# MatteoMer/zolt

Measured on AMD Instinct MI355X. Metric: BN254 G1 MSM/sec, higher is better.
Workload: dtype u32; 1 GPU; msm_g1_2^20; points=1048576, points_per_gpu=1048576, streams=3, window_bits=17, windows=15, table_levels=15, table_bytes=1006632960, mode=precomputed table of multiples

## Files before the change

### zolt_amd/csrc/msm.hip

```cpp
#include <string.h>

#include <mutex>
#include <vector>

#include "common.hip.h"
#include "g1.hip.h"
#include "g1_29.hip.h"
#include "g1_29x4.hip.h"
#include "msm_plan.h"

#ifndef ZG_TAIL_PRIO
#define ZG_TAIL_PRIO 3
#endif
#define ZG_HIPRIO() __builtin_amdgcn_s_setprio(ZG_TAIL_PRIO)

struct zg_bases_s {
    size_t n = 0;
    int device = -1;
    zg::MsmPlan plan;
    char *d_table = nullptr;
    uint8_t *d_inf = nullptr;
    uint64_t *d_scal = nullptr;
    struct Lane {
        uint32_t *d_dig = nullptr, *d_sorted = nullptr, *d_hist = nullptr, *d_starts = nullptr;
        uint32_t *d_blockhist = nullptr, *d_tmp = nullptr, *d_cstarts = nullptr, *d_fine = nullptr;
        zg::SortWords sort_cap;
        char *d_partial = nullptr;
        char *d_slice_buckets = nullptr;
        size_t slice_buckets = 0;
        uint32_t *d_slice_meta = nullptr;
        char *d_bits = nullptr;
        char *d_rg = nullptr;
        uint32_t *d_nzrank = nullptr;
        uint32_t *d_nzlist = nullptr;
        uint32_t *d_nzend = nullptr;
        uint32_t *d_scan_tmp = nullptr;
        char *d_part = nullptr;
        char *d_part2 = nullptr;
        uint32_t *d_heavy = nullptr;
        void *d_state = nullptr;
        hipEvent_t done = nullptr;
        hipStream_t last_st = nullptr;
        bool used = false;
    };
    std::vector<Lane> lanes;
    size_t next_lane = 0;
    Lane batch_lane;
    zg::MsmPlan batch_plan;
    size_t batch_n = 0;
    struct {
        size_t n = 0, k = 0, kc = 0;
        bool wide_ok = false;
    } fuse;
    static constexpr int NAUX = 3;
    hipStream_t aux[NAUX] = {nullptr, nullptr, nullptr};
    hipEvent_t ev_fork = nullptr, ev_join[NAUX] = {nullptr, nullptr, nullptr};
    zg_bases_s *small = nullptr;
    uint64_t *d_out = nullptr;
    uint64_t *h_out = nullptr;
    uint64_t *d_slice_parts = nullptr;
    char *d_rows_buckets = nullptr, *d_rows_bits = nullptr, *d_rows_rg = nullptr;
    size_t rows_cap = 0;
    hipEvent_t rows_done = nullptr;
    std::mutex mu;
};

namespace zg {


constexpr int PRE_GROUP = 7;
constexpr size_t PRE_CHUNK = (size_t)1 << 21;
struct PreJob {
    const uint64_t *xy;
    const uint8_t *inf;
    size_t n;
    int levels, dbl_per_level;
    char *table, *scratch;
    size_t first, count;
    unsigned blocks;
};
__global__ void __launch_bounds__(256) msm_precompute_kernel(PreJob side, PreJob main_job) {
    const bool is_side = blockIdx.x < side.blocks;
    const PreJob &jb = is_side ? side : main_job;
    const uint64_t *xy = jb.xy;
    const uint8_t *inf = jb.inf;
    const size_t n = jb.n, first = jb.first, count = jb.count;
    const int levels = jb.levels, dbl_per_level = jb.dbl_per_level;
    char *table = jb.table, *scratch = jb.scratch;
    const size_t li = (size_t)(blockIdx.x - (is_side ? 0u : side.blocks)) * blockDim.x + threadIdx.x, i = first + li;
    if (li >= count) return;
    Affine p = affine_load(xy + 8 * i);
    Jac29 a;
// ... 102 lines not shown
        __syncthreads();
    }
    if (k < NK) {
        loc[k] = sh[tid] - h;
        locz[k] = shz[tid] - z;
    }
    if (tid == 1023) {
        tile_tot[2 * blockIdx.x] = sh[1023];
        tile_tot[2 * blockIdx.x + 1] = shz[1023];
    }
}

__global__ void __launch_bounds__(1024) msm_scan_b_kernel(const uint32_t *__restrict__ hist, uint32_t NK, const uint32_t *__restrict__ loc,
                                                          const uint32_t *__restrict__ locz, const uint32_t *__restrict__ tile_tot,
                                                          uint32_t *__restrict__ starts, uint32_t *__restrict__ nzrank,
                                                          uint32_t *__restrict__ nzlist, uint32_t *__restrict__ nzend, uint32_t *__restrict__ state,
                                                          uint32_t nstate) {
    ZG_HIPRIO();
    __shared__ uint32_t pre[2];
    if (state && blockIdx.x == 0)
        for (uint32_t w = threadIdx.x; w < nstate; w += 1024) state[w] = 0;
    uint32_t tid = threadIdx.x, k = blockIdx.x * 1024 + tid;
    if (tid < 64) {
        uint32_t a = 0, az = 0;
        for (uint32_t t = tid; t < blockIdx.x; t += 64) {
            a += tile_tot[2 * t];
            az += tile_tot[2 * t + 1];
        }
        for (int d = 32; d > 0; d >>= 1) {
            a += __shfl_down(a, d, 64);
            az += __shfl_down(az, d, 64);
        }
        if (tid == 0) {
            pre[0] = a;
            pre[1] = az;
        }
    }
    __syncthreads();
    if (k < NK) {
        uint32_t s = pre[0] + loc[k], r = pre[1] + locz[k];
        starts[k] = s;
        nzrank[k] = r;
        uint32_t h = hist[k];
        if (h) {
            nzlist[r] = k;
            nzend[r] = s + h;
        }
        if (k == NK - 1) {
            starts[NK] = s + h;
            nzrank[NK] = r + (h ? 1u : 0u);
        }
    }
}

__global__ void __launch_bounds__(256) msm_scatter_kernel(const uint32_t *dig, uint32_t n, uint32_t n_pts, int G, size_t table_n,
                                                          uint32_t off, const uint32_t *starts, uint32_t *fill, uint32_t *sorted) {
    uint32_t i = blockIdx.x * 256 + threadIdx.x;
    uint32_t w = blockIdx.y;
    if (i >= n) return;
    uint32_t e = dig[(size_t)w * n + i];
    if (e == 0xFFFFFFFFu) return;
    uint32_t key = e & 0x7FFFFFFFu;
    uint32_t pos = starts[key] + atomicAdd(&fill[key], 1u);
    uint32_t ref = (uint32_t)((size_t)(w / G) * table_n + off + i % n_pts);
    sorted[pos] = (e & 0x80000000u) | ref;
}

struct RowOffs {
    uint32_t k;
    uint32_t off[33];
};
ZG_DEV void row_split(const RowOffs &r, uint32_t n_pts, uint32_t i, uint32_t &batch, uint32_t &pt) {
    if (r.k == 0) {
        batch = i / n_pts;
        pt = i - batch * n_pts;
        return;
    }
    uint32_t b = 0;
    while (b + 1 < r.k && i >= r.off[b + 1]) b++;
    batch = b;
    pt = i - r.off[b];
}

template <int C>
__global__ void __launch_bounds__(1024) msm_digits_lds_kernel(const uint64_t *scalars, const uint8_t *inf, uint32_t n, uint32_t n_pts,
                                                              int G, uint32_t per_block, uint32_t NK, int shift, uint32_t *dig,
                                                              uint32_t *blockhist, RowOffs rows) {
    ZG_HIPRIO();
    extern __shared__ uint32_t lds_hist[];
    constexpr int W = (255 + C - 1) / C;
    constexpr uint32_t NB = 1u << (C - 1);
    for (uint32_t k = threadIdx.x; k < NK; k += blockDim.x) lds_hist[k] = 0;
    __syncthreads();
    uint32_t i0 = blockIdx.x * per_block, i1 = i0 + per_block < n ? i0 + per_block : n;
    for (uint32_t i = i0 + threadIdx.x; i < i1; i += blockDim.x) {
        uint32_t batch, pt;
        row_split(rows, n_pts, i, batch, pt);
        Fr s = fr_from_mont29(fe_load<FrParams>(scalars + 4 * (rows.k ? (size_t)batch * n_pts + pt : (size_t)i)));
        bool skip = inf && inf[pt];
        uint32_t carry = 0;
#pragma unroll
        for (int w = 0; w < W; w++) {
            const int bit = w * C, limb = bit / 32, sh = bit % 32;
            uint32_t v = s.l[limb] >> sh;
            if (sh + C > 32 && limb + 1 < 8) v |= s.l[limb + 1] << (32 - sh);
            v = (v & ((1u << C) - 1u)) + carry;
            uint32_t neg = v > NB ? 1u : 0u;
            uint32_t d = neg ? (1u << C) - v : v;
            carry = neg;
            uint32_t e = 0xFFFFFFFFu;
            if (d != 0 && !skip) {
                uint32_t key = (batch * (uint32_t)G + (uint32_t)(w % G)) * NB + (d - 1);
                e = key | (neg << 31);
                atomicAdd(&lds_hist[key >> shift], 1u);
            }
            dig[(size_t)w * n + i] = e;
        }
    }
    __syncthreads();
    uint32_t *row = blockhist + (size_t)blockIdx.x * NK;
    for (uint32_t k = threadIdx.x; k < NK; k += blockDim.x) row[k] = lds_hist[k];
}

__global__ void __launch_bounds__(256) msm_colscan_kernel(uint32_t *blockhist, uint32_t nblk, uint32_t NK, uint32_t *total) {
    ZG_HIPRIO();
    uint32_t key = blockIdx.x * 256 + threadIdx.x;
    if (key >= NK) return;
    uint32_t run = 0;
    for (uint32_t b0 = 0; b0 < nblk; b0 += 16) {
        uint32_t v[16];
#pragma unroll
        for (int u = 0; u < 16; u++) v[u] = (b0 + u < nblk) ? blockhist[(size_t)(b0 + u) * NK + key] : 0u;
#pragma unroll
        for (int u = 0; u < 16; u++) {
            if (b0 + u < nblk) blockhist[(size_t)(b0 + u) * NK + key] = run;
            run += v[u];
        }
    }
    total[key] = run;
}

__global__ void __launch_bounds__(1024) msm_scatter_lds_kernel(const uint32_t *dig, uint32_t n, uint32_t n_pts, int W, int G,
                                                               size_t table_n, uint32_t off, uint32_t per_block, uint32_t NK,
                                                               const uint32_t *starts, const uint32_t *blockhist, uint32_t *sorted, RowOffs rows) {
    ZG_HIPRIO();
    extern __shared__ uint32_t lds_cur[];
    const uint32_t *row = blockhist + (size_t)blockIdx.x * NK;
    for (uint32_t k = threadIdx.x; k < NK; k += blockDim.x) lds_cur[k] = starts[k] + row[k];
    __syncthreads();
    uint32_t i0 = blockIdx.x * per_block, i1 = i0 + per_block < n ? i0 + per_block : n;
    if (i1 - i0 < blockDim.x) {
        const uint32_t cnt = i1 - i0, total = cnt * (uint32_t)W;
        for (uint32_t t = threadIdx.x; t < total; t += blockDim.x) {
            const uint32_t w = t / cnt, i = i0 + (t - w * cnt);
            uint32_t e = dig[(size_t)w * n + i];
            if (e == 0xFFFFFFFFu) continue;
            uint32_t pos = atomicAdd(&lds_cur[e & 0x7FFFFFFFu], 1u);
            uint32_t batch, pt;
            row_split(rows, n_pts, i, batch, pt);
            sorted[pos] = (e & 0x80000000u) | (uint32_t)((size_t)(w / (uint32_t)G) * table_n + off + pt);
        }
        return;
    }
    for (uint32_t i = i0 + threadIdx.x; i < i1; i += blockDim.x) {
        uint32_t batch, pt;
        row_split(rows, n_pts, i, batch, pt);
        for (int w0 = 0; w0 < W; w0 += 4) {
            uint32_t e[4];
#pragma unroll
            for (int u = 0; u < 4; u++) e[u] = w0 + u < W ? dig[(size_t)(w0 + u) * n + i] : 0xFFFFFFFFu;
#pragma unroll
            for (int u = 0; u < 4; u++) {
                if (e[u] == 0xFFFFFFFFu) continue;
                uint32_t pos = atomicAdd(&lds_cur[e[u] & 0x7FFFFFFFu], 1u);
                sorted[pos] = (e[u] & 0x80000000u) | (uint32_t)((size_t)((uint32_t)(w0 + u) / (uint32_t)G) * table_n + off + pt);
            }
        }
    }
}

__global__ void __launch_bounds__(1024) msm_coarse_base_kernel(const uint32_t *totals, uint32_t NCB, uint32_t *cstarts, uint32_t *tstarts,
                                                               uint32_t *istarts) {
    ZG_HIPRIO();
    __shared__ uint32_t sh[1024], sh4[1024], shi[1024];
    uint32_t tid = threadIdx.x, per = (NCB + 1023) / 1024, a = tid * per, b = a + per < NCB ? a + per : NCB;
    uint32_t s = 0, s4 = 0, si = 0;
    for (uint32_t k = a; k < b; k++) {
        s += totals[k];
        s4 += (totals[k] + 3u) & ~3u;
        si += (totals[k] + FINE_SLICE - 1) / FINE_SLICE;
    }
    sh[tid] = s;
    sh4[tid] = s4;
    shi[tid] = si;
    __syncthreads();
    for (uint32_t o = 1; o < 1024; o <<= 1) {
        uint32_t v = tid >= o ? sh[tid - o] : 0, v4 = tid >= o ? sh4[tid - o] : 0, vi = tid >= o ? shi[tid - o] : 0;
        __syncthreads();
        sh[tid] += v;
        sh4[tid] += v4;
        shi[tid] += vi;
        __syncthreads();
    }
    uint32_t run = sh[tid] - s, run4 = sh4[tid] - s4, runi = shi[tid] - si;
    for (uint32_t k = a; k < b; k++) {
        cstarts[k] = run;
        tstarts[k] = run4;
        istarts[k] = runi;
        run += totals[k];
        run4 += (totals[k] + 3u) & ~3u;
        runi += (totals[k] + FINE_SLICE - 1) / FINE_SLICE;
    }
    if (tid == 1023) {
        cstarts[NCB] = sh[1023];
        tstarts[NCB] = sh4[1023];
        istarts[NCB] = shi[1023];
    }
}

static constexpr uint32_t STAGE_ENTRIES = 32768;
template <bool PLAIN>
__global__ void __launch_bounds__(1024) msm_partition_kernel(const uint32_t *dig, uint32_t n, uint32_t n_pts, int W, int G, size_t table_n,
                                                             uint32_t off, uint32_t per_block, uint32_t NCB, int fb, int rb,
                                                             const uint32_t *tstarts, const uint32_t *blockoff, uint32_t *tmp, int local_shift,
                                                             RowOffs rows) {
    ZG_HIPRIO();
    extern __shared__ uint32_t lds[];
    uint32_t *buf = lds, *cnt = lds + STAGE_ENTRIES, *lbase = cnt + NCB, *sums = lbase + NCB + 1;
    const uint32_t tid = threadIdx.x, T = 1024, fmask = (1u << fb) - 1u;
    uint32_t i0 = blockIdx.x * per_block, cntl = i0 < n ? (n - i0 < per_block ? n - i0 : per_block) : 0;
    for (uint32_t k = tid; k < NCB; k += T) cnt[k] = 0;
    __syncthreads();
    const uint32_t jw2 = cntl > T ? 1u : 0u;
    uint32_t e[STAGE_ENTRIES / 1024];
#pragma unroll
    for (int r = 0; r < (int)(STAGE_ENTRIES / 1024); r++) {
        uint32_t w = (uint32_t)r >> jw2, j = ((uint32_t)r & jw2) * T + tid;
        e[r] = 0xFFFFFFFFu;
        if (w < (uint32_t)W && j < cntl) {
            uint32_t d = dig[(size_t)w * n + i0 + j];
            e[r] = d;
            if (d != 0xFFFFFFFFu) atomicAdd(&cnt[(d & 0x7FFFFFFFu) >> fb], 1u);
        }
    }
    __syncthreads();
    {
        uint32_t per = (NCB + T - 1) / T, a = tid * per, b = a + per < NCB ? a + per : NCB, sacc = 0;
        for (uint32_t k = a; k < b && k < NCB; k++) sacc += cnt[k];
        sums[tid] = sacc;
        __syncthreads();
        for (uint32_t o = 1; o < T; o <<= 1) {
            uint32_t v = tid >= o ? sums[tid - o] : 0;
            __syncthreads();
            sums[tid] += v;
            __syncthreads();
        }
        uint32_t run = sums[tid] - sacc;
        for (uint32_t k = a; k < b && k < NCB; k++) {
            lbase[k] = run;
            run += cnt[k];
            cnt[k] = 0;
        }
        if (tid == T - 1) lbase[NCB] = sums[T - 1];
    }
    __syncthreads();
    const uint32_t *row = blockoff + (size_t)blockIdx.x * NCB;
    uint32_t dst_pre[3];
#pragma unroll
    for (int u = 0; u < 3; u++) {
        uint32_t k = (uint32_t)u * T + tid;
        dst_pre[u] = k < NCB ? tstarts[k] + row[k] : 0u;
    }
    uint32_t pt_row0 = i0 + tid, pt_row1 = i0 + T + tid, row_unused;
    if (!PLAIN) {
        row_split(rows, n_pts, i0 + tid, row_unused, pt_row0);
        row_split(rows, n_pts, i0 + T + tid, row_unused, pt_row1);
    }
#pragma unroll
    for (int r = 0; r < (int)(STAGE_ENTRIES / 1024); r++) {
        if (e[r] != 0xFFFFFFFFu) {
            uint32_t w = (uint32_t)r >> jw2;
            uint32_t key = e[r] & 0x7FFFFFFFu, bin = key >> fb, lvl = (PLAIN || G == 1) ? w : w / (uint32_t)G;
            uint32_t pt = ((uint32_t)r & jw2) ? pt_row1 : pt_row0;
            const uint32_t ref = local_shift ? (lvl << local_shift) | pt : (uint32_t)((size_t)lvl * table_n + off + pt);
            uint32_t packed = (e[r] & 0x80000000u) | ((key & fmask) << rb) | ref;
            buf[lbase[bin] + atomicAdd(&cnt[bin], 1u)] = packed;
        }
    }
    __syncthreads();
#pragma unroll
    for (int u = 0; u < 3; u++) {
        uint32_t k = (uint32_t)u * T + tid;
        if (k < NCB) cnt[k] = dst_pre[u];
    }
    __syncthreads();
    const uint32_t avg = STAGE_ENTRIES / NCB, sg = avg >= 48 ? 64u : (avg >= 24 ? 32u : 16u), per = 64u / sg;
    const uint32_t lane = tid & 63, sub = lane / sg, sl = lane % sg;
    for (uint32_t bin = (tid >> 6) * per + sub; bin < NCB; bin += (T >> 6) * per) {
        uint32_t a = lbase[bin], b = lbase[bin + 1];
        uint32_t dst = cnt[bin];
        for (uint32_t j = a + sl; j < b; j += sg) tmp[dst + (j - a)] = buf[j];
    }
}

ZG_DEV bool fine_item(uint32_t item, const uint32_t *istarts, uint32_t NCB, uint32_t &bin, uint32_t &q0) {
    if (item >= istarts[NCB]) return false;
    uint32_t lo = 0, hi = NCB;
    while (hi - lo > 1) {
        uint32_t mid = (lo + hi) >> 1;
        if (istarts[mid] <= item) lo = mid; else hi = mid;
    }
    bin = lo;
    q0 = (item - istarts[lo]) * FINE_SLICE;
    return true;
}

__global__ void __launch_bounds__(1024) msm_fine_count_kernel(const uint32_t *tmp, const uint32_t *cstarts, const uint32_t *tstarts,
                                                              const uint32_t *istarts, uint32_t NCB, int fb, int rb, uint32_t *slicecnt) {
    ZG_HIPRIO();
    __shared__ uint32_t cnt[128];
    __shared__ uint32_t sh_bin, sh_q0, sh_ok;
    uint32_t tid = threadIdx.x, nf = 1u << fb, fmask = nf - 1u;
    if (tid == 0) {
        uint32_t bb = 0, qq = 0;
        sh_ok = fine_item(blockIdx.x, istarts, NCB, bb, qq) ? 1u : 0u;
        sh_bin = bb;
        sh_q0 = qq;
    }
    if (tid < nf) cnt[tid] = 0;
    __syncthreads();
    if (!sh_ok) return;
    uint32_t bin = sh_bin, q0 = sh_q0;
    uint32_t total = cstarts[bin + 1] - cstarts[bin];
    uint32_t count = total - q0 < FINE_SLICE ? total - q0 : FINE_SLICE;
    const uint4 *src = reinterpret_cast<const uint4 *>(tmp + tstarts[bin] + q0);
    const uint32_t T = blockDim.x, quads = (count + 3) / 4;
    for (uint32_t qb = 0; qb < quads; qb += 2 * T) {
        uint4 v[2];
#pragma unroll
        for (int u = 0; u < 2; u++) {
            uint32_t q = qb + u * T + tid;
            v[u] = q < quads ? src[q] : make_uint4(0, 0, 0, 0);
        }
#pragma unroll
        for (int u = 0; u < 2; u++) {
            uint32_t q = qb + u * T + tid, e[4] = {v[u].x, v[u].y, v[u].z, v[u].w};
#pragma unroll
            for (int j = 0; j < 4; j++)
                if (4 * q + j < count) atomicAdd(&cnt[(e[j] >> rb) & fmask], 1u);
        }
    }
    __syncthreads();
    if (tid < nf) slicecnt[(size_t)blockIdx.x * nf + tid] = cnt[tid];
}

__global__ void __launch_bounds__(1024) msm_fine_place_kernel(const uint32_t *tmp, const uint32_t *cstarts, const uint32_t *tstarts,
                                                              const uint32_t *istarts, uint32_t NCB, int fb, int rb, const uint32_t *slicecnt,
                                                              const uint32_t *fbase, uint32_t *sorted, int local_shift, uint32_t table_n,
                                                              uint32_t off) {
    ZG_HIPRIO();
    extern __shared__ uint32_t lds[];
    uint32_t *buf = lds, *cnt = lds + STAGE_ENTRIES, *lbase = cnt + 128;
    __shared__ uint32_t sh_bin, sh_q0, sh_ok;
    uint32_t tid = threadIdx.x, nf = 1u << fb, fmask = nf - 1u, rmask = (1u << rb) - 1u;
    if (tid == 0) {
        uint32_t bb = 0, qq = 0;
        sh_ok = fine_item(blockIdx.x, istarts, NCB, bb, qq) ? 1u : 0u;
        sh_bin = bb;
        sh_q0 = qq;
    }
    if (tid < nf) cnt[tid] = 0;
    __syncthreads();
    if (!sh_ok) return;
    uint32_t bin = sh_bin, q0 = sh_q0;
    uint32_t total = cstarts[bin + 1] - cstarts[bin];
    uint32_t count = total - q0 < FINE_SLICE ? total - q0 : FINE_SLICE;
    const uint4 *src = reinterpret_cast<const uint4 *>(tmp + tstarts[bin] + q0);
    const uint32_t T = 1024, quads = (count + 3) / 4;
    uint32_t dst_pre = tid < nf ? cstarts[bin] + fbase[(size_t)bin * nf + tid] + slicecnt[(size_t)blockIdx.x * nf + tid] : 0u;
    uint4 v[FINE_SLICE / 4 / 1024];
#pragma unroll
    for (int u = 0; u < (int)(FINE_SLICE / 4 / 1024); u++) {
        uint32_t q = (uint32_t)u * T + tid;
        v[u] = q < quads ? src[q] : make_uint4(0, 0, 0, 0);
    }
#pragma unroll
    for (int u = 0; u < (int)(FINE_SLICE / 4 / 1024); u++) {
        uint32_t q = (uint32_t)u * T + tid, e[4] = {v[u].x, v[u].y, v[u].z, v[u].w};
#pragma unroll
        for (int j = 0; j < 4; j++)
            if (4 * q + j < count) atomicAdd(&cnt[(e[j] >> rb) & fmask], 1u);
    }
    __syncthreads();
    if (tid == 0) {
        uint32_t run = 0;
        for (uint32_t f = 0; f < nf; f++) {
            lbase[f] = run;
            run += cnt[f];
            cnt[f] = 0;
        }
        lbase[nf] = run;
    }
    __syncthreads();
#pragma unroll
    for (int u = 0; u < (int)(FINE_SLICE / 4 / 1024); u++) {
        uint32_t q = (uint32_t)u * T + tid, e[4] = {v[u].x, v[u].y, v[u].z, v[u].w};
#pragma unroll
        for (int j = 0; j < 4; j++)
            if (4 * q + j < count) {
                uint32_t f = (e[j] >> rb) & fmask;
                uint32_t ref = e[j] & rmask;
                if (local_shift) ref = (ref >> local_shift) * table_n + off + (ref & ((1u << local_shift) - 1u));
                buf[lbase[f] + atomicAdd(&cnt[f], 1u)] = (e[j] & 0x80000000u) | ref;
            }
    }
    __syncthreads();
    if (tid < nf) cnt[tid] = dst_pre;
    __syncthreads();
    for (uint32_t f = tid >> 6; f < nf; f += T >> 6) {
        uint32_t a = lbase[f], b = lbase[f + 1];
        uint32_t dst = cnt[f];
        for (uint32_t j = a + (tid & 63); j < b; j += 64) sorted[dst + (j - a)] = buf[j];
    }
}

__global__ void __launch_bounds__(128) msm_fine_offsets_kernel(const uint32_t *istarts, int fb, uint32_t NK, uint32_t *slicecnt, uint32_t *fbase,
                                                               uint32_t *hist) {
    ZG_HIPRIO();
    __shared__ uint32_t sh[128];
    uint32_t bin = blockIdx.x, f = threadIdx.x, nf = 1u << fb;
    uint32_t i0 = istarts[bin], i1 = istarts[bin + 1], run = 0;
    if (f < nf)
        for (uint32_t it = i0; it < i1; it++) {
            uint32_t v = slicecnt[(size_t)it * nf + f];
            slicecnt[(size_t)it * nf + f] = run;
            run += v;
        }
    sh[f] = f < nf ? run : 0;
    __syncthreads();
    for (uint32_t o = 1; o < 128; o <<= 1) {
        uint32_t v = f >= o ? sh[f - o] : 0;
        __syncthreads();
        sh[f] += v;
        __syncthreads();
    }
    if (f < nf) {
        fbase[(size_t)bin * nf + f] = sh[f] - run;
        uint32_t key = (bin << fb) | f;
        if (key < NK) hist[key] = run;
    }
}

__global__ void __launch_bounds__(1024) msm_colscan_bins_kernel(uint32_t *chist, uint32_t nblk, uint32_t NCB, uint32_t *total) {
    ZG_HIPRIO();
    __shared__ uint32_t sh[64][16];
    const uint32_t lane = threadIdx.x & 15, slice = threadIdx.x >> 4, bin = blockIdx.x * 16 + lane;
    const uint32_t per = (nblk + 63) / 64, a = slice * per < nblk ? slice * per : nblk, b = a + per < nblk ? a + per : nblk;
    uint32_t s = 0;
    if (bin < NCB)
        for (uint32_t k = a; k < b; k++) s += chist[(size_t)k * NCB + bin];
    sh[slice][lane] = s;
    __syncthreads();
    uint32_t run = 0;
    for (uint32_t q = 0; q < slice; q++) run += sh[q][lane];
    if (bin < NCB) {
        for (uint32_t k = a; k < b; k++) {
            uint32_t v = chist[(size_t)k * NCB + bin];
            chist[(size_t)k * NCB + bin] = run;
            run += v;
        }
        if (slice == 63) total[bin] = run;
    }
}

// ... 781 lines not shown
    b->lanes.resize(nlanes);
    for (auto &ln : b->lanes) {
        hipError_t le = lane_alloc(ln, p, n);
        if (le != hipSuccess) {
            set_error(std::string("msm workspace: ") + hipGetErrorString(le));
            free_bases(b);
            return le == hipErrorOutOfMemory ? ZG_ERR_NOMEM : ZG_ERR_HIP;
        }
    }
    ZG_ALLOC(b->d_out, 16 * 8);
    if (hipHostMalloc((void **)&b->h_out, 16 * 8) != hipSuccess) {
        set_error("hipHostMalloc failed");
        free_bases(b);
        return ZG_ERR_NOMEM;
    }
    const bool want_small = !defer_table && (size_t)p.NB * p.G > 4096 && n > SIDE_TABLE_POINTS && env_int("ZG_MSM_SIDE_TABLE", 1);
    if (want_small) {
        zg_msm_config small_cfg{8, 0, 0};
        int src = bases_create(d_xy, d_inf_in, SIDE_TABLE_POINTS, &small_cfg, st, &b->small, true);
        if (src != ZG_OK) {
            b->small = nullptr;
            free_bases(b);
            return src;
        }
    }
    if (defer_table) {
        *out = b;
        return ZG_OK;
    }
    const size_t pre_levels = p.L > 1 ? (size_t)(p.L - 1 < PRE_GROUP ? p.L - 1 : PRE_GROUP) : 0;
    const size_t pre_chunk = n < PRE_CHUNK ? (n ? n : 1) : PRE_CHUNK;
    const bool v1 = env_int("ZG_MSM_PRECOMPUTE_V1", 0) != 0;
    Staging sg(st);
    char *pre_rec = n && pre_levels && !v1 ? sg.try_out<char>(pre_levels * pre_chunk * 144) : nullptr;
    const zg_bases_s *sm = b->small;
    char *side_rec = sm && !v1 ? sg.try_out<char>((size_t)PRE_GROUP * sm->n * 144) : nullptr;
    if (n) {
        if (d_inf_in) ZG_STAGE(sg, hipMemcpyAsync(b->d_inf, d_inf_in, n, hipMemcpyDeviceToDevice, st));
        if (sg.ok() && sm && d_inf_in) ZG_STAGE(sg, hipMemcpyAsync(sm->d_inf, d_inf_in, sm->n, hipMemcpyDeviceToDevice, st));
        if (sg.ok()) {
            PreJob side{};
            bool side_pending = sm != nullptr;
            if (side_pending && side_rec)
                side = PreJob{d_xy, sm->d_inf, sm->n, sm->plan.L, sm->plan.c * sm->plan.G, sm->d_table, side_rec, 0, sm->n, (unsigned)div_up(sm->n, 256)};
            if (pre_rec || p.L == 1) {
                for (size_t first = 0; first < n; first += pre_chunk) {
                    const size_t count = n - first < pre_chunk ? n - first : pre_chunk;
                    const PreJob mj{d_xy, b->d_inf, n, p.L, p.c * p.G, b->d_table, pre_rec, first, count, (unsigned)div_up(count, 256)};
                    hipLaunchKernelGGL(msm_precompute_kernel, dim3(side.blocks + mj.blocks), dim3(256), 0, st, side, mj);
                    if (side.blocks) side_pending = false;
                    side = PreJob{};
                }
            } else {
                hipLaunchKernelGGL(msm_precompute_v1_kernel, dim3(div_up(n, 256)), dim3(256), 0, st, d_xy, b->d_inf, n, p.L, p.c * p.G, b->d_table);
            }
            if (side_pending)
                hipLaunchKernelGGL(msm_precompute_v1_kernel, dim3(div_up(sm->n, 256)), dim3(256), 0, st, d_xy, sm->d_inf, sm->n, sm->plan.L,
                                   sm->plan.c * sm->plan.G, sm->d_table);
            sg.launched();
        }
    }
    if (sg.finish() != ZG_OK) {
        free_bases(b);
        return sg.rc;
    }
    *out = b;
    return ZG_OK;
}

template <int C>
static void launch_digits(hipStream_t st, const uint64_t *sc, const uint8_t *inf, uint32_t n, uint32_t n_pts, int G, uint32_t *dig,
                          uint32_t *hist) {
    hipLaunchKernelGGL(msm_digits_kernel<C>, dim3(div_up(n, 256)), dim3(256), 0, st, sc, inf, n, n_pts, G, dig, hist);
}

static unsigned sort_threads() {
    static const unsigned t = [] {
        int v = env_int("ZG_MSM_SORT_THREADS", 512);
        return (unsigned)(v >= 1024 ? 1024 : (v >= 512 ? 512 : 256));
    }();
    return t;
}

template <int C>
static int launch_digits_lds(hipStream_t st, const uint64_t *sc, const uint8_t *inf, uint32_t n, uint32_t n_pts, int G, uint32_t per_block,
                             uint32_t NK, uint32_t nblk, uint32_t *dig, uint32_t *blockhist, int shift, unsigned threads, const RowOffs &rows) {
    static PerDeviceOnce once;
    ZG_HIP(once.run([] {
        return hipFuncSetAttribute(reinterpret_cast<const void *>(msm_digits_lds_kernel<C>), hipFuncAttributeMaxDynamicSharedMemorySize, 128 * 1024);
    }));
    hipLaunchKernelGGL(msm_digits_lds_kernel<C>, dim3(nblk), dim3(threads), NK * 4, st, sc, inf, n, n_pts, G, per_block, NK, shift, dig, blockhist, rows);
    return ZG_OK;
}

static int launch_digits_lds_c(int c, hipStream_t st, const uint64_t *sc, const uint8_t *inf, uint32_t n, uint32_t n_pts, int G,
                               uint32_t per_block, uint32_t NK, uint32_t nblk, uint32_t *dig, uint32_t *blockhist, int shift = 0,
                               unsigned threads = 0, const RowOffs *rows_in = nullptr) {
    static const RowOffs uniform{};
    const RowOffs &rows = rows_in ? *rows_in : uniform;
    if (!threads) threads = sort_threads();
    switch (c) {
#define ZG_CASE(C) case C: return launch_digits_lds<C>(st, sc, inf, n, n_pts, G, per_block, NK, nblk, dig, blockhist, shift, threads, rows);
        ZG_CASE(2) ZG_CASE(3) ZG_CASE(4) ZG_CASE(5) ZG_CASE(6) ZG_CASE(7) ZG_CASE(8) ZG_CASE(9) ZG_CASE(10)
        ZG_CASE(11) ZG_CASE(12) ZG_CASE(13) ZG_CASE(14) ZG_CASE(15) ZG_CASE(16) ZG_CASE(17) ZG_CASE(18) ZG_CASE(19)
#undef ZG_CASE
        default: return invalid("msm: unsupported window size");
    }
}

static int launch_digits_c(int c, hipStream_t st, const uint64_t *sc, const uint8_t *inf, uint32_t n, uint32_t n_pts, int G, uint32_t *dig,
                           uint32_t *hist) {
    switch (c) {
#define ZG_CASE(C) case C: launch_digits<C>(st, sc, inf, n, n_pts, G, dig, hist); break;
        ZG_CASE(2) ZG_CASE(3) ZG_CASE(4) ZG_CASE(5) ZG_CASE(6) ZG_CASE(7) ZG_CASE(8) ZG_CASE(9) ZG_CASE(10)
        ZG_CASE(11) ZG_CASE(12) ZG_CASE(13) ZG_CASE(14) ZG_CASE(15) ZG_CASE(16) ZG_CASE(17) ZG_CASE(18) ZG_CASE(19)
#undef ZG_CASE
        default: return invalid("msm: unsupported window size");
    }
    return ZG_OK;
}

static int two_pass_attrs() {
    static PerDeviceOnce once;
    ZG_HIP(once.run([] {
        hipError_t err = hipFuncSetAttribute(reinterpret_cast<const void *>(msm_partition_kernel<true>), hipFuncAttributeMaxDynamicSharedMemorySize, 156 * 1024);
        if (err == hipSuccess)
            err = hipFuncSetAttribute(reinterpret_cast<const void *>(msm_partition_kernel<false>), hipFuncAttributeMaxDynamicSharedMemorySize, 156 * 1024);
        if (err == hipSuccess)
            err = hipFuncSetAttribute(reinterpret_cast<const void *>(msm_fine_place_kernel), hipFuncAttributeMaxDynamicSharedMemorySize, 156 * 1024);
        return err;
    }));
    return ZG_OK;
}

static int msm_enqueue_lane(zg_bases_s *b, const MsmPlan &p, zg_bases_s::Lane &ln, size_t off, size_t n_pts,
                            const uint64_t *d_scalars, hipStream_t st, int mode, uint64_t *d_rec, uint8_t *d_inf_out,
                            uint32_t rec_stride, uint32_t inf_stride);

static int ensure_aux_streams(zg_bases_s *b) {
    if (b->aux[0]) return ZG_OK;
    hipError_t e = hipEventCreateWithFlags(&b->ev_fork, hipEventDisableTiming);
    for (int i = 0; i < zg_bases_s::NAUX && e == hipSuccess; i++) {
        e = hipStreamCreateWithFlags(&b->aux[i], hipStreamNonBlocking);
        if (e == hipSuccess) e = hipEventCreateWithFlags(&b->ev_join[i], hipEventDisableTiming);
    }
    if (e != hipSuccess) {
        set_error(std::string("msm helper streams: ") + hipGetErrorString(e));
        return ZG_ERR_HIP;
    }
    return ZG_OK;
}

static size_t table_span_points(const zg_bases_s *b) { return table_span_points(b->plan.L); }
struct SliceView {
    uint32_t *sorted, *starts, *nzrank, *nzlist, *nzend;
    void *state;
};

__global__ void __launch_bounds__(256) msm_bucket_fold_kernel(char *buckets, const char *sets, uint32_t NK, uint32_t S) {
    ZG_HIPRIO();
    uint32_t k = (blockIdx.x * 256 + threadIdx.x) >> 2, q = threadIdx.x & 3;
    if (k >= NK) return;
    XYZZ29 acc = xyzz29_load(buckets + 144 * (size_t)k);
    XYZZ29 nxt = xyzz29_load(sets + 144 * (size_t)k);
    for (uint32_t j = 1; j < S; j++) {
        XYZZ29 cur = nxt;
        if (j + 1 < S) nxt = xyzz29_load(sets + 144 * ((size_t)j * NK + k));
        acc = xyzz29_add4(acc, cur, q);
    }
    if (q == 0) xyzz29_store(buckets + 144 * (size_t)k, acc);
}

static int msm_enqueue(zg_bases_s *b, size_t off, size_t n, const uint64_t *d_scalars, hipStream_t st, int mode, uint64_t *d_rec,
                       uint8_t *d_inf_out) {
    if (off + n > b->n) return invalid("msm: range exceeds uploaded bases");
    if (n == 0) {
        hipLaunchKernelGGL(msm_identity_kernel, dim3(1), dim3(1), 0, st, mode, d_rec, d_inf_out);
        ZG_HIP(hipGetLastError());
        return ZG_OK;
    }
    if (b->small && off + n <= b->small->n) return msm_enqueue(b->small, off, n, d_scalars, st, mode, d_rec, d_inf_out);
    zg_bases_s::Lane &ln = b->lanes[b->next_lane];
    b->next_lane = (b->next_lane + 1) % b->lanes.size();
    return msm_enqueue_lane(b, b->plan, ln, off, n, d_scalars, st, mode, d_rec, d_inf_out, 0, 0);
}

static thread_local const RowOffs *t_row_offs = nullptr;
static thread_local char *t_bucket_sink = nullptr;

static int msm_enqueue_lane(zg_bases_s *b, const MsmPlan &p, zg_bases_s::Lane &ln, size_t off, size_t n_pts,
                            const uint64_t *d_scalars, hipStream_t st, int mode, uint64_t *d_rec, uint8_t *d_inf_out,
                            uint32_t rec_stride, uint32_t inf_stride) {
    if (ln.used) ZG_HIP(hipStreamWaitEvent(st, ln.done, 0));
    ln.used = true;
    ln.last_st = st;
    size_t S, per;
    slice_counts(p, n_pts, S, per);
    MsmPlan ps = p;
    int local_shift = 0;
    if (S > 1 && slice_sort_plan(p, per, ps, local_shift) && !sort_words(ps, per).fit_in(ln.sort_cap)) {
        ps = p;
        local_shift = 0;
    }
    const size_t meta_stride = (4 * ((size_t)p.NK + 1) + state_words(p.NT, p.NK) + 3) & ~(size_t)3;
    if (S > 1 && ln.slice_buckets < S - 1) {
        if (ln.d_slice_buckets || ln.d_slice_meta) ZG_HIP(hipDeviceSynchronize());
        pool_free(ln.d_slice_buckets);
        ln.d_slice_buckets = nullptr;
        ln.slice_buckets = 0;
        ZG_HIP(lane_malloc((void **)&ln.d_slice_buckets, (S - 1) * (size_t)p.NK * 144));
        pool_free(ln.d_slice_meta);
        ln.d_slice_meta = nullptr;
        ZG_HIP(lane_malloc((void **)&ln.d_slice_meta, S * meta_stride * 4));
        ln.slice_buckets = S - 1;
    }
    auto sort_range = [&](size_t off, size_t n_pts, const uint64_t *d_scalars, const SliceView &sv) -> int {
    const MsmPlan &q = local_shift ? ps : p;
    const RowOffs *rows = t_row_offs && S == 1 && t_row_offs->k == (uint32_t)p.K && q.sort != MsmSort::ATOMIC ? t_row_offs : nullptr;
    static const RowOffs uniform_rows{};
    const RowOffs &rowv = rows ? *rows : uniform_rows;
    const size_t n = rows ? rows->off[rows->k] : n_pts * (size_t)p.K;
    const uint8_t *infp = b->d_inf ? b->d_inf + off : nullptr;
    const uint32_t nblk = sort_blocks(q, n);
    if (q.sort == MsmSort::TWO_PASS) {
        if ((size_t)nblk * q.NCB > ln.sort_cap.blockhist) return invalid("msm: two-pass workspace too small for this launch");
        uint32_t per_block = (uint32_t)((n + nblk - 1) / nblk);
        prof_begin(ZG_PROF_MSM_DIGITS, st);
        ZG_TRY(launch_digits_lds_c(p.c, st, d_scalars, infp, (uint32_t)n, (uint32_t)n_pts, p.G, per_block, q.NCB, nblk, ln.d_dig,
                                   ln.d_blockhist, q.fb, 256, rows));
        prof_end(ZG_PROF_MSM_DIGITS, st);
        prof_begin(ZG_PROF_MSM_SORT, st);
        uint32_t *d_tot = ln.d_cstarts + q.NCB + 1, *d_tst = ln.d_cstarts + 2 * (size_t)q.NCB + 2, *d_ist = ln.d_cstarts + 3 * (size_t)q.NCB + 3;
        hipLaunchKernelGGL(msm_colscan_bins_kernel, dim3(div_up(q.NCB, 16)), dim3(1024), 0, st, ln.d_blockhist, nblk, q.NCB, d_tot);
        hipLaunchKernelGGL(msm_coarse_base_kernel, dim3(1), dim3(1024), 0, st, d_tot, q.NCB, ln.d_cstarts, d_tst, d_ist);
        ZG_TRY(two_pass_attrs());
        if (!rows && p.G == 1 && n == n_pts)
            hipLaunchKernelGGL(msm_partition_kernel<true>, dim3(nblk), dim3(1024), (STAGE_ENTRIES + 2 * (size_t)q.NCB + 1 + 1024) * 4, st, ln.d_dig,
                               (uint32_t)n, (uint32_t)n_pts, p.W, p.G, b->n, (uint32_t)off, per_block, q.NCB, q.fb, q.rb, d_tst, ln.d_blockhist,
                               ln.d_tmp, local_shift, rowv);
        else
            hipLaunchKernelGGL(msm_partition_kernel<false>, dim3(nblk), dim3(1024), (STAGE_ENTRIES + 2 * (size_t)q.NCB + 1 + 1024) * 4, st, ln.d_dig,
                               (uint32_t)n, (uint32_t)n_pts, p.W, p.G, b->n, (uint32_t)off, per_block, q.NCB, q.fb, q.rb, d_tst, ln.d_blockhist,
                               ln.d_tmp, local_shift, rowv);
        {
            uint32_t items = (uint32_t)fine_max_items(q, n);
            uint32_t *d_fbase = ln.d_fine + (size_t)items * ((size_t)1 << q.fb);
            hipLaunchKernelGGL(msm_fine_count_kernel, dim3(items), dim3(1024), 0, st, ln.d_tmp, ln.d_cstarts, d_tst, d_ist, q.NCB, q.fb, q.rb,
                               ln.d_fine);
            hipLaunchKernelGGL(msm_fine_offsets_kernel, dim3(q.NCB), dim3(128), 0, st, d_ist, q.fb, p.NK, ln.d_fine, d_fbase, ln.d_hist);
            hipLaunchKernelGGL(msm_fine_place_kernel, dim3(items), dim3(1024), (STAGE_ENTRIES + 128 + 132) * 4, st, ln.d_tmp, ln.d_cstarts, d_tst,
                               d_ist, q.NCB, q.fb, q.rb, ln.d_fine, d_fbase, sv.sorted, local_shift, (uint32_t)b->n, (uint32_t)off);
        }
        uint32_t tiles = div_up(p.NK, 1024);
        hipLaunchKernelGGL(msm_scan_a_kernel, dim3(tiles), dim3(1024), 0, st, ln.d_hist, p.NK, ln.d_scan_tmp, ln.d_scan_tmp + p.NK,
                           ln.d_scan_tmp + 2 * (size_t)p.NK);
        hipLaunchKernelGGL(msm_scan_b_kernel, dim3(tiles), dim3(1024), 0, st, ln.d_hist, p.NK, ln.d_scan_tmp, ln.d_scan_tmp + p.NK,
                           ln.d_scan_tmp + 2 * (size_t)p.NK, sv.starts, sv.nzrank, sv.nzlist, sv.nzend, reinterpret_cast<uint32_t *>(sv.state),
                           state_words(p.NT, p.NK));
    } else if (q.sort == MsmSort::LDS) {
        uint32_t per_block = (uint32_t)((n + nblk - 1) / nblk);
        prof_begin(ZG_PROF_MSM_DIGITS, st);
        ZG_TRY(launch_digits_lds_c(p.c, st, d_scalars, infp, (uint32_t)n, (uint32_t)n_pts, p.G, per_block, p.NK, nblk, ln.d_dig,
                                   ln.d_blockhist, 0, 0, rows));
        prof_end(ZG_PROF_MSM_DIGITS, st);
        prof_begin(ZG_PROF_MSM_SORT, st);
        hipLaunchKernelGGL(msm_colscan_kernel, dim3(div_up(p.NK, 256)), dim3(256), 0, st, ln.d_blockhist, nblk, p.NK, ln.d_hist);
        {
            uint32_t tiles = div_up(p.NK, 1024);
            hipLaunchKernelGGL(msm_scan_a_kernel, dim3(tiles), dim3(1024), 0, st, ln.d_hist, p.NK, ln.d_scan_tmp, ln.d_scan_tmp + p.NK,
                               ln.d_scan_tmp + 2 * (size_t)p.NK);
            hipLaunchKernelGGL(msm_scan_b_kernel, dim3(tiles), dim3(1024), 0, st, ln.d_hist, p.NK, ln.d_scan_tmp, ln.d_scan_tmp + p.NK,
                               ln.d_scan_tmp + 2 * (size_t)p.NK, sv.starts, sv.nzrank, sv.nzlist, sv.nzend, reinterpret_cast<uint32_t *>(sv.state),
                               state_words(p.NT, p.NK));
        }
        static PerDeviceOnce scatter_once;
        ZG_HIP(scatter_once.run([] {
            return hipFuncSetAttribute(reinterpret_cast<const void *>(msm_scatter_lds_kernel), hipFuncAttributeMaxDynamicSharedMemorySize, 128 * 1024);
        }));
        hipLaunchKernelGGL(msm_scatter_lds_kernel, dim3(nblk), dim3(sort_threads()), p.NK * 4, st, ln.d_dig, (uint32_t)n, (uint32_t)n_pts, p.W, p.G,
                           b->n, (uint32_t)off, per_block, p.NK, sv.starts, ln.d_blockhist, sv.sorted, rowv);
    } else {
        prof_begin(ZG_PROF_MSM_DIGITS, st);
        ZG_HIP(hipMemsetAsync(ln.d_hist, 0, (size_t)p.NK * 4, st));
        ZG_TRY(launch_digits_c(p.c, st, d_scalars, infp, (uint32_t)n, (uint32_t)n_pts, p.G, ln.d_dig, ln.d_hist));
        prof_end(ZG_PROF_MSM_DIGITS, st);
        prof_begin(ZG_PROF_MSM_SORT, st);
        {
            uint32_t tiles = div_up(p.NK, 1024);
            hipLaunchKernelGGL(msm_scan_a_kernel, dim3(tiles), dim3(1024), 0, st, ln.d_hist, p.NK, ln.d_scan_tmp, ln.d_scan_tmp + p.NK,
                               ln.d_scan_tmp + 2 * (size_t)p.NK);
            hipLaunchKernelGGL(msm_scan_b_kernel, dim3(tiles), dim3(1024), 0, st, ln.d_hist, p.NK, ln.d_scan_tmp, ln.d_scan_tmp + p.NK,
                               ln.d_scan_tmp + 2 * (size_t)p.NK, sv.starts, sv.nzrank, sv.nzlist, sv.nzend, reinterpret_cast<uint32_t *>(sv.state),
                               state_words(p.NT, p.NK));
        }
        ZG_HIP(hipMemsetAsync(ln.d_hist, 0, (size_t)p.NK * 4, st));
        hipLaunchKernelGGL(msm_scatter_kernel, dim3(div_up(n, 256), p.W), dim3(256), 0, st, ln.d_dig, (uint32_t)n, (uint32_t)n_pts, p.G,
                           b->n, (uint32_t)off, sv.starts, ln.d_hist, sv.sorted);
    }
    prof_end(ZG_PROF_MSM_SORT, st);
    return ZG_OK;
    };
    auto accumulate_range = [&](size_t n_pts, const SliceView &sv, char *bucket_out) -> int {
    const size_t n = n_pts * (size_t)p.K;
    prof_begin(ZG_PROF_MSM_ACCUMULATE, st);
    bool alone = env_int("ZG_MSM_ALONE_FULL", 1) != 0;
    for (auto &o : b->lanes)
        if (alone && &o != &ln && o.used && o.last_st != st && hipEventQuery(o.done) == hipErrorNotReady) alone = false;
    (void)hipGetLastError();
    if (p.G > 1) alone = true;
    uint32_t NT = chunk_threads((uint64_t)n * p.W, alone);
    if (NT > p.NT || forced_chunk_threads()) NT = p.NT;
    static const unsigned acc_block = [] {
        int v = env_int("ZG_MSM_ACC_BLOCK", 256);
        return (unsigned)(v == 64 || v == 128 ? v : 256);
    }();
#ifdef ZG_ACC_RUNEND_STARTS
    const uint32_t *run_ends = sv.nzlist;
#else
    const uint32_t *run_ends = sv.nzend;
#endif
    if (NT <= (uint32_t)env_int("ZG_MSM_QUAD_ACC_MAX_CHUNKS", 32768))
        hipLaunchKernelGGL(msm_accumulate_chunk_kernel<true>, dim3(div_up((size_t)NT * 4, 256)), dim3(256), 0, st, sv.sorted, sv.starts,
                           sv.nzrank, run_ends, b->d_table, p.NK, NT, ln.d_part);
    else
        hipLaunchKernelGGL(msm_accumulate_chunk_kernel<false>, dim3(div_up(NT, acc_block)), dim3(acc_block), 0, st, sv.sorted, sv.starts,
                           sv.nzrank, run_ends, b->d_table, p.NK, NT, ln.d_part);
    prof_end(ZG_PROF_MSM_ACCUMULATE, st);
    prof_begin(ZG_PROF_MSM_REDUCE, st);
    if (p.tail == MsmTail::LANE)
        hipLaunchKernelGGL(msm_bucket_combine_lane_kernel, dim3(div_up(p.NK, 64)), dim3(64), 0, st, ln.d_part, sv.starts, sv.nzrank, p.NK, NT,
                           bucket_out, ln.d_heavy, reinterpret_cast<MsmState *>(sv.state));
    else
        hipLaunchKernelGGL(msm_bucket_combine_kernel, dim3(div_up((size_t)p.NK * p.GS * 4, 64)), dim3(64), 0, st, ln.d_part, sv.starts,
                           sv.nzrank, p.NK, NT, p.GS, bucket_out, ln.d_heavy, reinterpret_cast<MsmState *>(sv.state));
// ... 607 lines not shown
```

Baseline: 861.4 MSM/s.

## Derive sort bin counts from prefix offsets and add plain digit kernel path

```diff
diff --git a/zolt_amd/csrc/msm.hip b/zolt_amd/csrc/msm.hip
--- a/zolt_amd/csrc/msm.hip
+++ b/zolt_amd/csrc/msm.hip
@@ -8,6 +8,7 @@
 #include "g1_29.hip.h"
 #include "g1_29x4.hip.h"
 #include "msm_plan.h"
+#include "msm_sort_walk.h"
 
 #ifndef ZG_TAIL_PRIO
 #define ZG_TAIL_PRIO 3
@@ -276,7 +277,7 @@
     pt = i - r.off[b];
 }
 
-template <int C>
+template <int C, bool PLAIN>
 __global__ void __launch_bounds__(1024) msm_digits_lds_kernel(const uint64_t *scalars, const uint8_t *inf, uint32_t n, uint32_t n_pts,
                                                               int G, uint32_t per_block, uint32_t NK, int shift, uint32_t *dig,
                                                               uint32_t *blockhist, RowOffs rows) {
@@ -288,11 +289,12 @@
     __syncthreads();
     uint32_t i0 = blockIdx.x * per_block, i1 = i0 + per_block < n ? i0 + per_block : n;
     for (uint32_t i = i0 + threadIdx.x; i < i1; i += blockDim.x) {
-        uint32_t batch, pt;
-        row_split(rows, n_pts, i, batch, pt);
-        Fr s = fr_from_mont29(fe_load<FrParams>(scalars + 4 * (rows.k ? (size_t)batch * n_pts + pt : (size_t)i)));
-        bool skip = inf && inf[pt];
+        uint32_t batch = 0, pt = i;
+        if (!PLAIN) row_split(rows, n_pts, i, batch, pt);
+        Fr s = fr_from_mont29(fe_load<FrParams>(scalars + 4 * (!PLAIN && rows.k ? (size_t)batch * n_pts + pt : (size_t)i)));
+        const bool skip = !PLAIN && inf && inf[pt];
         uint32_t carry = 0;
+        uint32_t *out = dig + i;
 #pragma unroll
         for (int w = 0; w < W; w++) {
             const int bit = w * C, limb = bit / 32, sh = bit % 32;
@@ -304,11 +306,16 @@
             carry = neg;
             uint32_t e = 0xFFFFFFFFu;
             if (d != 0 && !skip) {
-                uint32_t key = (batch * (uint32_t)G + (uint32_t)(w % G)) * NB + (d - 1);
+                uint32_t key = PLAIN ? d - 1 : (batch * (uint32_t)G + (uint32_t)(w % G)) * NB + (d - 1);
                 e = key | (neg << 31);
                 atomicAdd(&lds_hist[key >> shift], 1u);
             }
-            dig[(size_t)w * n + i] = e;
+            if (PLAIN) {
+                *out = e;
+                out += n;
+            } else {
+                dig[(size_t)w * n + i] = e;
+            }
         }
     }
     __syncthreads();
@@ -416,15 +423,26 @@
 template <bool PLAIN>
 __global__ void __launch_bounds__(1024) msm_partition_kernel(const uint32_t *dig, uint32_t n, uint32_t n_pts, int W, int G, size_t table_n,
                                                              uint32_t off, uint32_t per_block, uint32_t NCB, int fb, int rb,
-                                                             const uint32_t *tstarts, const uint32_t *blockoff, uint32_t *tmp, int local_shift,
-                                                             RowOffs rows) {
+                                                             const uint32_t *tstarts, const uint32_t *blockoff, const uint32_t *totals,
+                                                             uint32_t *tmp, int local_shift, RowOffs rows) {
     ZG_HIPRIO();
     extern __shared__ uint32_t lds[];
     uint32_t *buf = lds, *cnt = lds + STAGE_ENTRIES, *lbase = cnt + NCB, *sums = lbase + NCB + 1;
     const uint32_t tid = threadIdx.x, T = 1024, fmask = (1u << fb) - 1u;
     uint32_t i0 = blockIdx.x * per_block, cntl = i0 < n ? (n - i0 < per_block ? n - i0 : per_block) : 0;
-    for (uint32_t k = tid; k < NCB; k += T) cnt[k] = 0;
-    __syncthreads();
+    const uint32_t *row = blockoff + (size_t)blockIdx.x * NCB;
+    const uint32_t *nxt = blockIdx.x + 1 == gridDim.x ? totals : row + NCB;
+    uint32_t dst_pre[3];
+#pragma unroll
+    for (int u = 0; u < 3; u++) {
+        uint32_t k = (uint32_t)u * T + tid;
+        dst_pre[u] = 0u;
+        if (k < NCB) {
+            const uint32_t own = row[k];
+            cnt[k] = sort_walk::count_of(own, nxt[k]);
+            dst_pre[u] = tstarts[k] + own;
+        }
+    }
     const uint32_t jw2 = cntl > T ? 1u : 0u;
     uint32_t e[STAGE_ENTRIES / 1024];
 #pragma unroll
@@ -434,7 +452,6 @@
         if (w < (uint32_t)W && j < cntl) {
             uint32_t d = dig[(size_t)w * n + i0 + j];
             e[r] = d;
-            if (d != 0xFFFFFFFFu) atomicAdd(&cnt[(d & 0x7FFFFFFFu) >> fb], 1u);
         }
     }
     __syncthreads();
@@ -458,13 +475,6 @@
         if (tid == T - 1) lbase[NCB] = sums[T - 1];
     }
     __syncthreads();
-    const uint32_t *row = blockoff + (size_t)blockIdx.x * NCB;
-    uint32_t dst_pre[3];
-#pragma unroll
-    for (int u = 0; u < 3; u++) {
-        uint32_t k = (uint32_t)u * T + tid;
-        dst_pre[u] = k < NCB ? tstarts[k] + row[k] : 0u;
-    }
     uint32_t pt_row0 = i0 + tid, pt_row1 = i0 + T + tid, row_unused;
     if (!PLAIN) {
         row_split(rows, n_pts, i0 + tid, row_unused, pt_row0);
@@ -488,13 +498,7 @@
         if (k < NCB) cnt[k] = dst_pre[u];
     }
     __syncthreads();
-    const uint32_t avg = STAGE_ENTRIES / NCB, sg = avg >= 48 ? 64u : (avg >= 24 ? 32u : 16u), per = 64u / sg;
-    const uint32_t lane = tid & 63, sub = lane / sg, sl = lane % sg;
-    for (uint32_t bin = (tid >> 6) * per + sub; bin < NCB; bin += (T >> 6) * per) {
-        uint32_t a = lbase[bin], b = lbase[bin + 1];
-        uint32_t dst = cnt[bin];
-        for (uint32_t j = a + sl; j < b; j += sg) tmp[dst + (j - a)] = buf[j];
-    }
+    sort_walk::copy_out(lbase, cnt, NCB, tid >> 6, tid & 63, [&](uint32_t j, uint32_t pos) { tmp[pos] = buf[j]; });
 }
 
 ZG_DEV bool fine_item(uint32_t item, const uint32_t *istarts, uint32_t NCB, uint32_t &bin, uint32_t &q0) {
@@ -550,8 +554,8 @@
 
 __global__ void __launch_bounds__(1024) msm_fine_place_kernel(const uint32_t *tmp, const uint32_t *cstarts, const uint32_t *tstarts,
                                                               const uint32_t *istarts, uint32_t NCB, int fb, int rb, const uint32_t *slicecnt,
-                                                              const uint32_t *fbase, uint32_t *sorted, int local_shift, uint32_t table_n,
-                                                              uint32_t off) {
+                                                              const uint32_t *fbase, const uint32_t *hist, uint32_t NK, uint32_t *sorted,
+                                                              int local_shift, uint32_t table_n, uint32_t off) {
     ZG_HIPRIO();
     extern __shared__ uint32_t lds[];
     uint32_t *buf = lds, *cnt = lds + STAGE_ENTRIES, *lbase = cnt + 128;
@@ -563,7 +567,6 @@
         sh_bin = bb;
         sh_q0 = qq;
     }
-    if (tid < nf) cnt[tid] = 0;
     __syncthreads();
     if (!sh_ok) return;
     uint32_t bin = sh_bin, q0 = sh_q0;
@@ -571,19 +574,19 @@
     uint32_t count = total - q0 < FINE_SLICE ? total - q0 : FINE_SLICE;
     const uint4 *src = reinterpret_cast<const uint4 *>(tmp + tstarts[bin] + q0);
     const uint32_t T = 1024, quads = (count + 3) / 4;
-    uint32_t dst_pre = tid < nf ? cstarts[bin] + fbase[(size_t)bin * nf + tid] + slicecnt[(size_t)blockIdx.x * nf + tid] : 0u;
+    const bool last = blockIdx.x + 1 == istarts[bin + 1];
+    uint32_t dst_pre = 0u;
+    if (tid < nf) {
+        const uint32_t own = slicecnt[(size_t)blockIdx.x * nf + tid], key = (bin << fb) | tid;
+        const uint32_t next = last ? (key < NK ? hist[key] : own) : slicecnt[((size_t)blockIdx.x + 1) * nf + tid];
+        cnt[tid] = sort_walk::count_of(own, next);
+        dst_pre = cstarts[bin] + fbase[(size_t)bin * nf + tid] + own;
+    }
     uint4 v[FINE_SLICE / 4 / 1024];
 #pragma unroll
     for (int u = 0; u < (int)(FINE_SLICE / 4 / 1024); u++) {
         uint32_t q = (uint32_t)u * T + tid;
         v[u] = q < quads ? src[q] : make_uint4(0, 0, 0, 0);
-    }
-#pragma unroll
-    for (int u = 0; u < (int)(FINE_SLICE / 4 / 1024); u++) {
-        uint32_t q = (uint32_t)u * T + tid, e[4] = {v[u].x, v[u].y, v[u].z, v[u].w};
-#pragma unroll
-        for (int j = 0; j < 4; j++)
-            if (4 * q + j < count) atomicAdd(&cnt[(e[j] >> rb) & fmask], 1u);
     }
     __syncthreads();
     if (tid == 0) {
@@ -1531,25 +1534,30 @@
     return t;
 }
 
-template <int C>
+template <int C, bool PLAIN>
 static int launch_digits_lds(hipStream_t st, const uint64_t *sc, const uint8_t *inf, uint32_t n, uint32_t n_pts, int G, uint32_t per_block,
                              uint32_t NK, uint32_t nblk, uint32_t *dig, uint32_t *blockhist, int shift, unsigned threads, const RowOffs &rows) {
     static PerDeviceOnce once;
     ZG_HIP(once.run([] {
-        return hipFuncSetAttribute(reinterpret_cast<const void *>(msm_digits_lds_kernel<C>), hipFuncAttributeMaxDynamicSharedMemorySize, 128 * 1024);
+        return hipFuncSetAttribute(reinterpret_cast<const void *>(msm_digits_lds_kernel<C, PLAIN>), hipFuncAttributeMaxDynamicSharedMemorySize,
+                                   128 * 1024);
     }));
-    hipLaunchKernelGGL(msm_digits_lds_kernel<C>, dim3(nblk), dim3(threads), NK * 4, st, sc, inf, n, n_pts, G, per_block, NK, shift, dig, blockhist, rows);
+    hipLaunchKernelGGL((msm_digits_lds_kernel<C, PLAIN>), dim3(nblk), dim3(threads), NK * 4, st, sc, inf, n, n_pts, G, per_block, NK, shift, dig,
+                       blockhist, rows);
     return ZG_OK;
 }
 
 static int launch_digits_lds_c(int c, hipStream_t st, const uint64_t *sc, const uint8_t *inf, uint32_t n, uint32_t n_pts, int G,
                                uint32_t per_block, uint32_t NK, uint32_t nblk, uint32_t *dig, uint32_t *blockhist, int shift = 0,
-                               unsigned threads = 0, const RowOffs *rows_in = nullptr) {
+                               unsigned threads = 0, const RowOffs *rows_in = nullptr, bool plain = false) {
     static const RowOffs uniform{};
     const RowOffs &rows = rows_in ? *rows_in : uniform;
     if (!threads) threads = sort_threads();
     switch (c) {
-#define ZG_CASE(C) case C: return launch_digits_lds<C>(st, sc, inf, n, n_pts, G, per_block, NK, nblk, dig, blockhist, shift, threads, rows);
+#define ZG_CASE(C)                                                                                                                        \
+    case C:                                                                                                                               \
+        if (C >= 14 && plain) return launch_digits_lds<C, (C >= 14)>(st, sc, nullptr, n, n_pts, G, per_block, NK, nblk, dig, blockhist, shift, threads, rows); \
+        return launch_digits_lds<C, false>(st, sc, inf, n, n_pts, G, per_block, NK, nblk, dig, blockhist, shift, threads, rows);
         ZG_CASE(2) ZG_CASE(3) ZG_CASE(4) ZG_CASE(5) ZG_CASE(6) ZG_CASE(7) ZG_CASE(8) ZG_CASE(9) ZG_CASE(10)
         ZG_CASE(11) ZG_CASE(12) ZG_CASE(13) ZG_CASE(14) ZG_CASE(15) ZG_CASE(16) ZG_CASE(17) ZG_CASE(18) ZG_CASE(19)
 #undef ZG_CASE
@@ -1674,23 +1682,24 @@
     if (q.sort == MsmSort::TWO_PASS) {
         if ((size_t)nblk * q.NCB > ln.sort_cap.blockhist) return invalid("msm: two-pass workspace too small for this launch");
         uint32_t per_block = (uint32_t)((n + nblk - 1) / nblk);
+        const bool plain = !rows && p.G == 1 && n == n_pts;
         prof_begin(ZG_PROF_MSM_DIGITS, st);
         ZG_TRY(launch_digits_lds_c(p.c, st, d_scalars, infp, (uint32_t)n, (uint32_t)n_pts, p.G, per_block, q.NCB, nblk, ln.d_dig,
-                                   ln.d_blockhist, q.fb, 256, rows));
+                                   ln.d_blockhist, q.fb, 256, rows, plain && !infp));
         prof_end(ZG_PROF_MSM_DIGITS, st);
         prof_begin(ZG_PROF_MSM_SORT, st);
         uint32_t *d_tot = ln.d_cstarts + q.NCB + 1, *d_tst = ln.d_cstarts + 2 * (size_t)q.NCB + 2, *d_ist = ln.d_cstarts + 3 * (size_t)q.NCB + 3;
         hipLaunchKernelGGL(msm_colscan_bins_kernel, dim3(div_up(q.NCB, 16)), dim3(1024), 0, st, ln.d_blockhist, nblk, q.NCB, d_tot);
         hipLaunchKernelGGL(msm_coarse_base_kernel, dim3(1), dim3(1024), 0, st, d_tot, q.NCB, ln.d_cstarts, d_tst, d_ist);
         ZG_TRY(two_pass_attrs());
-        if (!rows && p.G == 1 && n == n_pts)
+        if (plain)
             hipLaunchKernelGGL(msm_partition_kernel<true>, dim3(nblk), dim3(1024), (STAGE_ENTRIES + 2 * (size_t)q.NCB + 1 + 1024) * 4, st, ln.d_dig,
                                (uint32_t)n, (uint32_t)n_pts, p.W, p.G, b->n, (uint32_t)off, per_block, q.NCB, q.fb, q.rb, d_tst, ln.d_blockhist,
-                               ln.d_tmp, local_shift, rowv);
+                               d_tot, ln.d_tmp, local_shift, rowv);
         else
             hipLaunchKernelGGL(msm_partition_kernel<false>, dim3(nblk), dim3(1024), (STAGE_ENTRIES + 2 * (size_t)q.NCB + 1 + 1024) * 4, st, ln.d_dig,
                                (uint32_t)n, (uint32_t)n_pts, p.W, p.G, b->n, (uint32_t)off, per_block, q.NCB, q.fb, q.rb, d_tst, ln.d_blockhist,
-                               ln.d_tmp, local_shift, rowv);
+                               d_tot, ln.d_tmp, local_shift, rowv);
         {
             uint32_t items = (uint32_t)fine_max_items(q, n);
             uint32_t *d_fbase = ln.d_fine + (size_t)items * ((size_t)1 << q.fb);
@@ -1698,7 +1707,7 @@
                                ln.d_fine);
             hipLaunchKernelGGL(msm_fine_offsets_kernel, dim3(q.NCB), dim3(128), 0, st, d_ist, q.fb, p.NK, ln.d_fine, d_fbase, ln.d_hist);
             hipLaunchKernelGGL(msm_fine_place_kernel, dim3(items), dim3(1024), (STAGE_ENTRIES + 128 + 132) * 4, st, ln.d_tmp, ln.d_cstarts, d_tst,
-                               d_ist, q.NCB, q.fb, q.rb, ln.d_fine, d_fbase, sv.sorted, local_shift, (uint32_t)b->n, (uint32_t)off);
+                               d_ist, q.NCB, q.fb, q.rb, ln.d_fine, d_fbase, ln.d_hist, p.NK, sv.sorted, local_shift, (uint32_t)b->n, (uint32_t)off);
         }
         uint32_t tiles = div_up(p.NK, 1024);
         hipLaunchKernelGGL(msm_scan_a_kernel, dim3(tiles), dim3(1024), 0, st, ln.d_hist, p.NK, ln.d_scan_tmp, ln.d_scan_tmp + p.NK,
diff --git a/zolt_amd/csrc/msm_sort_walk.h b/zolt_amd/csrc/msm_sort_walk.h
--- /dev/null
+++ b/zolt_amd/csrc/msm_sort_walk.h
@@ -0,0 +1,44 @@
+#pragma once
+#include <stdint.h>
+
+#if defined(__HIP__)
+#define ZG_SORT_WALK_FN __attribute__((host)) __attribute__((device)) inline
+#else
+#define ZG_SORT_WALK_FN inline
+#endif
+
+namespace zg {
+namespace sort_walk {
+
+static constexpr uint32_t WAVE = 64;
+static constexpr uint32_t WAVE_SPAN = 2048;
+
+ZG_SORT_WALK_FN uint32_t count_of(uint32_t own, uint32_t next) { return next - own; }
+
+ZG_SORT_WALK_FN uint32_t run_of(const uint32_t *lbase, uint32_t nbins, uint32_t j) {
+    uint32_t lo = 0, hi = nbins;
+    while (hi - lo > 1) {
+        uint32_t mid = (lo + hi) >> 1;
+        if (lbase[mid] <= j) lo = mid; else hi = mid;
+    }
+    return lo;
+}
+
+template <class Put>
+ZG_SORT_WALK_FN void copy_out(const uint32_t *lbase, const uint32_t *dst, uint32_t nbins, uint32_t wave, uint32_t lane, Put put) {
+    const uint32_t total = lbase[nbins];
+    uint32_t j = wave * WAVE_SPAN + lane;
+    if (j >= total) return;
+    uint32_t bin = run_of(lbase, nbins, j);
+    uint32_t end = lbase[bin + 1], shift = dst[bin] - lbase[bin];
+    for (uint32_t t = 0; t < WAVE_SPAN / WAVE && j < total; t++, j += WAVE) {
+        if (j >= end) {
+            do end = lbase[++bin + 1]; while (j >= end);
+            shift = dst[bin] - lbase[bin];
+        }
+        put(j, j + shift);
+    }
+}
+
+}
+}
```

Measured after the change: 866.4 MSM/s, median of 6. About the same (+0.6%).
